# mhpi/hydrodl2

Hardware: AMD Instinct MI355X
Metric: basin-ensemble-timesteps/sec fwd+bwd (higher is better)
Workload: dtype f32

## Files before the change

hydrodl2_amd/csrc/hbv_chunked.h:

```cpp
#pragma once

#include <hip/hip_runtime.h>

#include "../../include/hbvx.h"
#include "hbv_step.h"

namespace hbvx {

struct ChunkArgs {
    hbvx_desc d;
    hbvx_bwd_io io;
    int lgMp;
    int C;
    int nchunk;
    float *phi;
    float *abnd;
    float *gpart;
    int nd;
    int dslot[3];
    int per_xcd;
};

struct ChunkBlock {
    int bx, chunk;
};
__host__ __device__ inline int chunk_per_xcd(int B, int lgMp)
{
    const int bpw = 64 >> lgMp;
    return ((B + bpw - 1) / bpw + 7) / 8;
}
__device__ __forceinline__ bool chunk_block(const hbvx_desc &d, int lgMp, int per_xcd, ChunkBlock &b)
{
    const int i = blockIdx.x;
#if defined(HBVX_CHUNK_XCD) && HBVX_CHUNK_XCD == 0
    b.chunk = i / (8 * per_xcd);
    b.bx = i - b.chunk * (8 * per_xcd);
#else
    const int c = i & 7, k = i >> 3;
    b.chunk = k / per_xcd;
    b.bx = c * per_xcd + (k - b.chunk * per_xcd);
#endif
    return b.bx * (64 >> lgMp) < d.B;
}

#define CHUNK_FEW 3

template <int NP>
__device__ __forceinline__ void slot_set(float *p, int slot, float v)
{
#pragma unroll
    for (int i = 0; i < NP; i++)
        if (slot == i) p[i] = v;
}
template <int NP>
__device__ __forceinline__ float slot_get(const float *p, int slot)
{
    float v = 0.0f;
#pragma unroll
    for (int i = 0; i < NP; i++)
        if (slot == i) v = p[i];
    return v;
}

struct ChunkLane {
    int jm, b, j;
    bool active, leader;
    int64_t n;
};

__device__ __forceinline__ ChunkLane chunk_lane(const hbvx_desc &d, int lgMp, int bx)
{
    ChunkLane L;
    const int lane = threadIdx.x & 63;
    const int Mp = 1 << lgMp;
    L.jm = lane & (Mp - 1);
    int b = bx * (64 >> lgMp) + (lane >> lgMp);
    L.active = (b < d.B) && (L.jm < d.M);
    L.leader = (b < d.B) && (L.jm == 0);
    L.b = b < d.B ? b : d.B - 1;
    L.j = L.jm < d.M ? L.jm : d.M - 1;
    L.n = (int64_t)L.b * d.M + L.j;
    return L;
}

template <int MODEL, bool BETAET>
struct ChunkNP {
    static constexpr int value = MODEL == MODEL_HBV10 ? (BETAET ? 13 : 12)
                               : MODEL == MODEL_HBV11P ? 14 : (MODEL == MODEL_HOURLY ? 19 : 16);
};

template <int NP>
struct ChunkRaw {
    float f[3];
    float st[5];
    float sw0, ef0;
    float gf[HBVX_MAX_FLUX];
    float g4[4];
    float dv[NP];
    float mu;
};

template <int MODEL, bool BETAET, int NP>
struct ChunkDay {
// ... 199 lines not shown
    const int chunk = blk.chunk;
    const int t0 = chunk * A.C, t1 = min(d.T, t0 + A.C);
    const int64_t N = (int64_t)d.B * d.M;
    const bool raw = d.raw_sigmoid != 0;
    const float nz = d.nearzero, invM = 1.0f / (float)d.M;
    const float ac = (MODEL == MODEL_HBV20 || MODEL == MODEL_HOURLY) ? d.ac[L.b] : 0.0f;
    const float elev = (MODEL == MODEL_HBV20 || MODEL == MODEL_HOURLY) ? d.elev[L.b] : 0.0f;
    float usta[NP], psta[NP];
    bool use_dyn[NP];
    chunk_static<NP, DYN>(d, L, raw, usta, psta, use_dyn, nd_, ds_);

    float Phi[5][5], phi[5];
#pragma unroll
    for (int k = 0; k < 5; k++) {
        phi[k] = 0.0f;
#pragma unroll
        for (int i = 0; i < 5; i++) Phi[k][i] = (i == k) ? 1.0f : 0.0f;
    }
    FluxGrad g0;
    g0.gQ = g0.gQ0 = g0.gQ1 = g0.gQ2 = g0.gET = g0.gSWE = g0.grech = g0.gexc = g0.gef = g0.gtosoil =
        g0.gPERC = g0.gcap = 0.0f;
    constexpr bool LDSDV = DYN == 3;
    __shared__ float dvbuf[LDSDV ? NP * 64 : 1];
    ChunkRaw<NP> Rn;
    if (LDSDV) chunk_dma_dyn<NP>(d, L, t1 - 1, dvbuf);
    chunk_issue<NP, DYN, GFULL, LDSDV, MU>(d, io, L, t1 - 1, io.n_flux, Rn, nd_, ds_);
    for (int t = t1 - 1; t >= t0; t--) {
        ChunkRaw<NP> Rc = Rn;
        if (LDSDV) {
            asm volatile("s_waitcnt vmcnt(0)" ::: "memory");
            chunk_pull_dyn<NP>(Rc, dvbuf);
            asm volatile("s_waitcnt lgkmcnt(0)" ::: "memory");
        }
        if (t > t0) {
            if (LDSDV) chunk_dma_dyn<NP>(d, L, t - 1, dvbuf);
            chunk_issue<NP, DYN, GFULL, LDSDV, MU>(d, io, L, t - 1, io.n_flux, Rn, nd_, ds_);
        }
        ChunkDay<MODEL, BETAET, NP> D;
        chunk_finish<MODEL, BETAET, NP, DYN, GFULL, MU>(d, Rc, raw, nz, ac, elev, usta, psta, use_dyn,
                                                    io.n_flux, invM, D, nd_, ds_, io.grad_flux4 != nullptr);
        float gp[NPARAM_MAX], gx[3];
#pragma unroll
        for (int i = 0; i < NPARAM_MAX; i++) gp[i] = 0.0f;
        if constexpr (MODEL == MODEL_HBV10) {
            typedef Step<MODEL, BETAET> S;
            const typename S::JT c = D.s.jt_coef(D.p, nz);
            S::template jt_unit<0>(c, Phi[0]);
            S::template jt_unit<0>(c, Phi[1]);
            S::template jt_unit<1>(c, Phi[2]);
            S::template jt_unit<2>(c, Phi[3]);
            S::template jt_unit<2>(c, Phi[4]);
            if constexpr (!GFULL) {
                S::jt_affine(c, phi, D.g.gQ0 + D.g.gQ, D.g.gQ1 + D.g.gQ, D.g.gQ2 + D.g.gQ);
                continue;
            }
        } else if constexpr (MODEL == MODEL_HBV11P || MODEL == MODEL_HBV20) {
            typedef Step<MODEL, BETAET> S;
            const typename S::JTC c = D.s.jt_coef_cap(D.p, nz);
            S::template jt_unit<0>(c, Phi[0]);
            S::template jt_unit<0>(c, Phi[1]);
#pragma unroll
            for (int k = 2; k < 5; k++) S::jt_cap(c, Phi[k], 0.0f, 0.0f, 0.0f);
            if constexpr (!GFULL) {
                S::jt_cap(c, phi, D.g.gQ0 + D.g.gQ, D.g.gQ1 + D.g.gQ, D.g.gQ2 + D.g.gQ);
                continue;
            }
        } else {
#pragma unroll
            for (int k = 0; k < 5; k++) D.s.bwd(D.p, nz, g0, Phi[k], gp, gx);
        }
        D.s.bwd(D.p, nz, D.g, phi, gp, gx);
    }
    if (L.active) {
        float *dst = A.phi + ((int64_t)chunk * 30) * N + L.n;
#pragma unroll
        for (int k = 0; k < 5; k++)
#pragma unroll
            for (int i = 0; i < 5; i++) dst[(int64_t)(k * 5 + i) * N] = Phi[k][i];
#pragma unroll
        for (int i = 0; i < 5; i++) dst[(int64_t)(25 + i) * N] = phi[i];
    }
}

__host__ __device__ constexpr int onepass_kmin(int i)
{
    return (i == P_TT || i == P_CFMAX || i == P_CFR || i == P_CWH) ? 0
         : ((i == P_BETA || i == P_FC || i == P_LP || i == P_BETAET) ? 2 : 3);
}
__host__ __device__ constexpr int onepass_row(int i)
{
    int r = 0;
    for (int j = 0; j < i; j++) r += 6 - onepass_kmin(j);
    return r;
}
__host__ __device__ constexpr int onepass_rows(int NP) { return onepass_row(NP); }

template <bool BETAET, bool GFULL>
__global__ void __launch_bounds__(64) k_bwd_chunk_onepass(const ChunkArgs A)
{
    constexpr int MODEL = MODEL_HBV10, DYN = 0;
    constexpr int NP = ChunkNP<MODEL, BETAET>::value;
    typedef Step<MODEL, BETAET> S;
    const int ds_[3] = {0, 0, 0};
    const hbvx_desc &d = A.d;
    const hbvx_bwd_io &io = A.io;
    ChunkBlock blk;
    if (!chunk_block(d, A.lgMp, A.per_xcd, blk)) return;
    const ChunkLane L = chunk_lane(d, A.lgMp, blk.bx);
    const int chunk = blk.chunk;
    const int t0 = chunk * A.C, t1 = min(d.T, t0 + A.C);
    const int64_t N = (int64_t)d.B * d.M;
    const bool raw = d.raw_sigmoid != 0;
    const float nz = d.nearzero, invM = 1.0f / (float)d.M;
    float usta[NP], psta[NP];
    bool use_dyn[NP];
    chunk_static<NP, DYN>(d, L, raw, usta, psta, use_dyn, 0, ds_);

    float Phi[5][5], phi[5];
    float G[6][NPARAM_MAX];
#pragma unroll
    for (int k = 0; k < 5; k++) {
        phi[k] = 0.0f;
#pragma unroll
        for (int i = 0; i < 5; i++) Phi[k][i] = (i == k) ? 1.0f : 0.0f;
    }
#pragma unroll
    for (int k = 0; k < 6; k++)
#pragma unroll
        for (int i = 0; i < NPARAM_MAX; i++) G[k][i] = 0.0f;
    ChunkRaw<NP> Rn;
    chunk_issue<NP, DYN, GFULL>(d, io, L, t1 - 1, io.n_flux, Rn, 0, ds_);
    for (int t = t1 - 1; t >= t0; t--) {
        ChunkRaw<NP> Rc = Rn;
        if (t > t0) chunk_issue<NP, DYN, GFULL>(d, io, L, t - 1, io.n_flux, Rn, 0, ds_);
        ChunkDay<MODEL, BETAET, NP> D;
        chunk_finish<MODEL, BETAET, NP, DYN, GFULL>(d, Rc, raw, nz, 0.0f, 0.0f, usta, psta, use_dyn, io.n_flux, invM,
                                                    D, 0, ds_, io.grad_flux4 != nullptr);
        const typename S::JT c = D.s.jt_coef(D.p, nz);
        const typename S::JG k = D.s.jg_coef(D.p, nz);
        S::template jt_gp<0>(c, k, Phi[0], G[0]);
        S::template jt_gp<0>(c, k, Phi[1], G[1]);
        S::template jt_gp<1>(c, k, Phi[2], G[2]);
        S::template jt_gp<2>(c, k, Phi[3], G[3]);
        S::template jt_gp<2>(c, k, Phi[4], G[4]);
        if constexpr (!GFULL) {
            S::template jt_gp<2, true>(c, k, phi, G[5], D.g.gQ0 + D.g.gQ, D.g.gQ1 + D.g.gQ, D.g.gQ2 + D.g.gQ);
        } else {
            float gx[3];
            D.s.bwd(D.p, nz, D.g, phi, G[5], gx);
        }
    }
    if (L.active) {
        float *dst = A.phi + ((int64_t)chunk * 30) * N + L.n;
#pragma unroll
        for (int k = 0; k < 5; k++)
#pragma unroll
            for (int i = 0; i < 5; i++) dst[(int64_t)(k * 5 + i) * N] = Phi[k][i];
#pragma unroll
        for (int i = 0; i < 5; i++) dst[(int64_t)(25 + i) * N] = phi[i];
        float *gdst = A.gpart + ((int64_t)chunk * onepass_rows(NP)) * N + L.n;
#pragma unroll
        for (int i = 0; i < NP; i++) {
            const int r0 = onepass_row(i), k0 = onepass_kmin(i);
#pragma unroll
            for (int kk = 0; kk < 5; kk++)
                if (kk >= k0) gdst[(int64_t)(r0 + kk - k0) * N] = G[kk][i];
            gdst[(int64_t)(r0 + 5 - k0) * N] = G[5][i];
        }
    }
}

#ifndef HBVX_CHUNK_NO_SHARED_KERNELS
__global__ void __launch_bounds__(64) k_bwd_chunk_scan(const ChunkArgs A)
{
    const hbvx_desc &d = A.d;
    const int64_t N = (int64_t)d.B * d.M;
    const int64_t n = (int64_t)blockIdx.x * 64 + threadIdx.x;
    if (n >= N) return;
    float a[5];
#pragma unroll
    for (int k = 0; k < 5; k++) a[k] = A.io.grad_state_out ? A.io.grad_state_out[k * N + n] : 0.0f;
    constexpr int SCAN_DEPTH = 4;
    float buf[SCAN_DEPTH][30];
    auto fetch = [&](int c, float *dst) __attribute__((always_inline)) {
        const float *src = A.phi + ((int64_t)c * 30) * N + n;
#pragma unroll
        for (int i = 0; i < 30; i++) dst[i] = src[(int64_t)i * N];
    };
#pragma unroll
    for (int j = 0; j < SCAN_DEPTH; j++)
        if (A.nchunk - 1 - j >= 0) fetch(A.nchunk - 1 - j, buf[j]);
    for (int c0 = A.nchunk - 1; c0 >= 0; c0 -= SCAN_DEPTH) {
#pragma unroll
        for (int j = 0; j < SCAN_DEPTH; j++) {
            const int c = c0 - j;
            if (c < 0) break;
            float cur[30];
#pragma unroll
            for (int i = 0; i < 30; i++) cur[i] = buf[j][i];
            if (c - SCAN_DEPTH >= 0) fetch(c - SCAN_DEPTH, buf[j]);
#pragma unroll
            for (int k = 0; k < 5; k++) A.abnd[((int64_t)c * 5 + k) * N + n] = a[k];
            float an[5];
#pragma unroll
            for (int i = 0; i < 5; i++) {
                float v = cur[25 + i];
#pragma unroll
                for (int k = 0; k < 5; k++) v += a[k] * cur[k * 5 + i];
                an[i] = v;
            }
#pragma unroll
            for (int i = 0; i < 5; i++) a[i] = an[i];
        }
    }
    if (A.io.grad_state_in) {
#pragma unroll
        for (int k = 0; k < 5; k++) A.io.grad_state_in[k * N + n] = a[k];
    }
}

#endif

__device__ __forceinline__ float chunk_ens_sum(float v, int lgMp)
{
    for (int s = 0; s < lgMp; s++) v += __shfl_xor(v, 1 << s, 64);
    return v;
}

template <int MODEL, bool BETAET, int DYN, bool GFULL, int SC = 0, bool ROWST = false, bool MU = false>
__global__ void __launch_bounds__(64) k_bwd_chunk_sweep(const ChunkArgs A)
{
    CHUNK_SLOTS(A);
    constexpr int NP = ChunkNP<MODEL, BETAET>::value;
    __shared__ float rowbuf[ROWST ? 64 * NP : 1];
    const hbvx_desc &d = A.d;
    const hbvx_bwd_io &io = A.io;
    ChunkBlock blk;
    if (!chunk_block(d, A.lgMp, A.per_xcd, blk)) return;
    const ChunkLane L = chunk_lane(d, A.lgMp, blk.bx);
    const int chunk = blk.chunk;
    const int t0 = chunk * A.C, t1 = min(d.T, t0 + A.C);
    const int64_t N = (int64_t)d.B * d.M;
    const bool raw = d.raw_sigmoid != 0;
    const float nz = d.nearzero, invM = 1.0f / (float)d.M;
    const float ac = (MODEL == MODEL_HBV20 || MODEL == MODEL_HOURLY) ? d.ac[L.b] : 0.0f;
    const float elev = (MODEL == MODEL_HBV20 || MODEL == MODEL_HOURLY) ? d.elev[L.b] : 0.0f;
    float usta[NP], psta[NP], gsta[NP];
    bool use_dyn[NP];
    chunk_static<NP, DYN>(d, L, raw, usta, psta, use_dyn, nd_, ds_);
#pragma unroll
    for (int i = 0; i < NP; i++) gsta[i] = 0.0f;
// ... 54 lines not shown
            const int M = d.M, rowf = NP * M, bl = (threadIdx.x & 63) >> A.lgMp;
            if (L.jm < M) {
#pragma unroll
                for (int i = 0; i < NP; i++) {
                    const float gu = gp[i] * (d.p[i].hi - d.p[i].lo);
                    rowbuf[bl * rowf + i * M + L.jm] = raw ? gu * (D.ud[i] * (1.0f - D.ud[i])) : gu;
                }
            }
            const int b0 = blk.bx * (64 >> A.lgMp);
            const int nb = min(64 >> A.lgMp, d.B - b0);
            const int half = rowf >> 1, total2 = nb * half;
            float *gbase = io.g[0].dyn + (int64_t)t * io.g[0].dyn_t_stride + (int64_t)b0 * io.g[0].dyn_b_stride;
            for (int k = threadIdx.x & 63; k < total2; k += 64) {
                const int rb = k / half, w2 = k - rb * half;
                const float2 v = *reinterpret_cast<const float2 *>(&rowbuf[rb * rowf + 2 * w2]);
                *reinterpret_cast<float2 *>(gbase + (int64_t)rb * io.g[0].dyn_b_stride + 2 * w2) = v;
            }
        }
#pragma unroll
        for (int i = 0; i < NP; i++) {
            if (DYN == 1 || DYN == 3) break;
            const float gu = gp[i] * (d.p[i].hi - d.p[i].lo);
            if (DYN == 2) {
                const float gr = raw ? gu * (D.ud[i] * (1.0f - D.ud[i])) : gu;
                if (io.g[i].dyn && L.active)
                    io.g[i].dyn[(int64_t)t * io.g[i].dyn_t_stride + (int64_t)L.b * io.g[i].dyn_b_stride + L.j] =
                        use_dyn[i] ? gr : 0.0f;
                gsta[i] += use_dyn[i] ? 0.0f : gu;
            } else {
                gsta[i] += gu;
            }
        }
        if (io.grad_x) {
            const float act = L.active ? 1.0f : 0.0f;
            const float g0 = chunk_ens_sum(gx[0] * act, A.lgMp), g1 = chunk_ens_sum(gx[1] * act, A.lgMp),
                        g2 = chunk_ens_sum(gx[2] * act, A.lgMp);
            if (L.leader) {
                float *gr = io.grad_x + (int64_t)t * d.x_t_stride + (int64_t)L.b * d.x_b_stride;
                gr[d.ch_prcp] = g0; gr[d.ch_tmean] = g1; gr[d.ch_pet] = g2;
            }
        }
    }
    if (DYN == 1) {
#pragma unroll
        for (int k = 0; k < CHUNK_FEW; k++)
            if (k < nd_) slot_set<NP>(gsta, ds_[k], slot_get<NP>(gsta, ds_[k]) - gused[k]);
    }
    if (DYN != 3 && L.active) {
#pragma unroll
        for (int i = 0; i < NP; i++) A.gpart[((int64_t)chunk * NP + i) * N + L.n] = gsta[i];
    }
}

#ifndef HBVX_CHUNK_NO_SHARED_KERNELS
__global__ void __launch_bounds__(256) k_bwd_chunk_reduce(const ChunkArgs A, int NP)
{
    const hbvx_desc &d = A.d;
    const hbvx_bwd_io &io = A.io;
    const int64_t N = (int64_t)d.B * d.M;
    const int64_t n = (int64_t)blockIdx.x * 256 + threadIdx.x;
    const int i = blockIdx.y;
    if (n >= N || !io.g[i].sta) return;
    const float *src = A.gpart + (int64_t)i * N + n;
    const int64_t cs = (int64_t)NP * N;
    float acc0 = 0.0f, acc1 = 0.0f, acc2 = 0.0f, acc3 = 0.0f;
    int c = 0;
    for (; c + 3 < A.nchunk; c += 4) {
        acc0 += src[(int64_t)c * cs];
        acc1 += src[(int64_t)(c + 1) * cs];
        acc2 += src[(int64_t)(c + 2) * cs];
        acc3 += src[(int64_t)(c + 3) * cs];
    }
    for (; c < A.nchunk; c++) acc0 += src[(int64_t)c * cs];
    float gsum = (acc0 + acc1) + (acc2 + acc3);
    const int b = (int)(n / d.M), j = (int)(n % d.M);
    if (d.raw_sigmoid) {
        const float u = sigmoid_(d.p[i].sta[(int64_t)b * d.p[i].sta_b_stride + j]);
        gsum = gsum * (u * (1.0f - u));
    }
    float *dst = io.g[i].sta + (int64_t)b * io.g[i].sta_b_stride + j;
    *dst += gsum;
}

#define ONEPASS_GROUP 4
template <int NP>
__global__ void __launch_bounds__(256) k_bwd_chunk_fold(const ChunkArgs A)
{
    constexpr int NR = onepass_rows(NP);
    const hbvx_desc &d = A.d;
    const int64_t N = (int64_t)d.B * d.M;
    const int64_t n = (int64_t)blockIdx.x * 256 + threadIdx.x;
    if (n >= N) return;
    const int grp = blockIdx.y;
    const int c0 = grp * ONEPASS_GROUP, c1 = min(A.nchunk, c0 + ONEPASS_GROUP);
    double acc[NP];
#pragma unroll
    for (int i = 0; i < NP; i++) acc[i] = 0.0;
    for (int c = c0; c < c1; c++) {
        const float *g = A.gpart + (int64_t)c * NR * N + n;
        const float *ab = A.abnd + (int64_t)c * 5 * N + n;
        double a[5];
#pragma unroll
        for (int k = 0; k < 5; k++) a[k] = ab[(int64_t)k * N];
#pragma unroll
        for (int i = 0; i < NP; i++) {
            const int k0 = onepass_kmin(i), r0 = onepass_row(i);
            double v = g[(int64_t)(r0 + 5 - k0) * N];
#pragma unroll
            for (int k = 0; k < 5; k++)
                if (k >= k0) v += (double)g[(int64_t)(r0 + k - k0) * N] * a[k];
            acc[i] += v;
        }
    }
    float *dst = A.phi + (int64_t)grp * NP * N + n;
#pragma unroll
    for (int i = 0; i < NP; i++) dst[(int64_t)i * N] = (float)acc[i] * (d.p[i].hi - d.p[i].lo);
}

#endif

}
```

hydrodl2_amd/csrc/launch_chunked.hip:

```cpp
#include "hbvx_host.h"
#include "hbv_chunked.h"

#include <algorithm>
#include <atomic>

using namespace hbvx;
using namespace hbvx_host;

namespace hbvx_host {
void launch_chunk_scan(const hbvx::ChunkArgs &a, hipStream_t st)
{
    const int64_t N = (int64_t)a.d.B * a.d.M;
    hipLaunchKernelGGL(k_bwd_chunk_scan, dim3((unsigned)((N + 63) / 64)), dim3(64), 0, st, a);
}
void launch_chunk_reduce(const hbvx::ChunkArgs &a, int n_param, hipStream_t st)
{
    const int64_t N = (int64_t)a.d.B * a.d.M;
    hipLaunchKernelGGL(k_bwd_chunk_reduce, dim3((unsigned)((N + 255) / 256), n_param), dim3(256), 0, st, a, n_param);
}
}

int hbvx_host::chunk_days() { int c = env_int("HBVX_CHUNK", 64); return c < 2 ? 2 : c; }

bool hbvx_host::chunked_applicable(const hbvx_desc *d)
{
    const char *v = getenv("HBVX_BWD");
    if (v && !strcmp(v, "tiled")) return false;
    return d->T >= 2 * chunk_days();
}

static int np_of(const hbvx_desc *d) { return d->n_param; }

static bool onepass_admitted(const hbvx_desc *d)
{
    return d->model == HBVX_MODEL_HBV10 && (d->n_param == 12 || d->n_param == 13) && count_dyn(d) == 0;
}

static int gpart_rows(const hbvx_desc *d)
{
    const int np = np_of(d);
    return onepass_admitted(d) ? std::max(np, onepass_rows(np)) : np;
}

extern "C" uint64_t hbvx_backward_workspace_bytes(const hbvx_desc *d)
{
    if (!d || d->T <= 0 || d->B <= 0 || d->M <= 0 || !chunked_applicable(d)) return 0;
    const int C = chunk_days();
    const uint64_t nchunk = (uint64_t)(d->T + C - 1) / C;
    return nchunk * (uint64_t)d->B * (uint64_t)d->M * (uint64_t)(35 + gpart_rows(d)) * sizeof(float);
}

static std::atomic<int> g_chunk_form{0};
extern "C" int hbvx_chunk_form(void) { return g_chunk_form.load(); }

template <int MODEL, bool BETAET, int DYN, bool GFULL>
static hipError_t launch_chunked_t(const ChunkArgs &a, hipStream_t st, bool onepass)
{
    const hbvx_desc &d = a.d;
    const int bpw = 64 >> a.lgMp;
    const int64_t N = (int64_t)d.B * d.M;
    (void)bpw;
    dim3 g2((unsigned)(8 * a.per_xcd * a.nchunk));
    if constexpr (MODEL == MODEL_HBV10 && DYN == 0) {
        if (onepass) {
            g_chunk_form = 1;
            hipLaunchKernelGGL((k_bwd_chunk_onepass<BETAET, GFULL>), g2, dim3(64), 0, st, a);
            hipLaunchKernelGGL(k_bwd_chunk_scan, dim3((unsigned)((N + 63) / 64)), dim3(64), 0, st, a);
            store_gate(&a.io, st);
            const int ngroup = (a.nchunk + ONEPASS_GROUP - 1) / ONEPASS_GROUP;
            hipLaunchKernelGGL((k_bwd_chunk_fold<ChunkNP<MODEL, BETAET>::value>),
                               dim3((unsigned)((N + 255) / 256), (unsigned)ngroup), dim3(256), 0, st, a);
            ChunkArgs r = a;
            r.gpart = a.phi;
            r.nchunk = ngroup;
            hipLaunchKernelGGL(k_bwd_chunk_reduce, dim3((unsigned)((N + 255) / 256), d.n_param), dim3(256), 0, st,
                               r, d.n_param);
            return hipGetLastError();
        }
    }
    g_chunk_form = 2;
    int sc = 0;
    const bool mu = d.muwts != nullptr;
    if (!mu && DYN == 1 && MODEL == MODEL_HBV10 && BETAET && a.nd == 2 && a.dslot[0] == P_BETA && a.dslot[1] == P_BETAET) sc = 1;
    if (!mu && DYN == 1 && (MODEL == MODEL_HBV20 || MODEL == MODEL_HOURLY) && a.nd == 3 && a.dslot[0] == P_BETA &&
        a.dslot[1] == P_K0 && a.dslot[2] == P_BETAET)
        sc = 2;
    if constexpr (DYN == 1 && MODEL == MODEL_HBV10 && BETAET) {
        if (sc == 1) {
            hipLaunchKernelGGL((k_bwd_chunk_phi<MODEL, BETAET, DYN, GFULL, 1>), g2, dim3(64), 0, st, a);
            hipLaunchKernelGGL(k_bwd_chunk_scan, dim3((unsigned)((N + 63) / 64)), dim3(64), 0, st, a);
            store_gate(&a.io, st);
            hipLaunchKernelGGL((k_bwd_chunk_sweep<MODEL, BETAET, DYN, GFULL, 1>), g2, dim3(64), 0, st, a);
        }
    }
    if constexpr (DYN == 1 && (MODEL == MODEL_HBV20 || MODEL == MODEL_HOURLY)) {
        if (sc == 2) {
            hipLaunchKernelGGL((k_bwd_chunk_phi<MODEL, BETAET, DYN, GFULL, 2>), g2, dim3(64), 0, st, a);
            hipLaunchKernelGGL(k_bwd_chunk_scan, dim3((unsigned)((N + 63) / 64)), dim3(64), 0, st, a);
            store_gate(&a.io, st);
            hipLaunchKernelGGL((k_bwd_chunk_sweep<MODEL, BETAET, DYN, GFULL, 2>), g2, dim3(64), 0, st, a);
        }
    }
    if (sc != 0) {
        hipLaunchKernelGGL(k_bwd_chunk_reduce, dim3((unsigned)((N + 255) / 256), d.n_param), dim3(256), 0, st,
                           a, d.n_param);
        return hipGetLastError();
    }
    if constexpr (DYN == 0 || DYN == 1) {
        if (d.muwts) {
            hipLaunchKernelGGL((k_bwd_chunk_phi<MODEL, BETAET, DYN, GFULL, 0, true>), g2, dim3(64), 0, st, a);
            hipLaunchKernelGGL(k_bwd_chunk_scan, dim3((unsigned)((N + 63) / 64)), dim3(64), 0, st, a);
            store_gate(&a.io, st);
            hipLaunchKernelGGL((k_bwd_chunk_sweep<MODEL, BETAET, DYN, GFULL, 0, false, true>), g2, dim3(64), 0, st, a);
            hipLaunchKernelGGL(k_bwd_chunk_reduce, dim3((unsigned)((N + 255) / 256), d.n_param), dim3(256), 0, st,
                               a, d.n_param);
            return hipGetLastError();
        }
    }
    hipLaunchKernelGGL((k_bwd_chunk_phi<MODEL, BETAET, DYN, GFULL>), g2, dim3(64), 0, st, a);
    hipLaunchKernelGGL(k_bwd_chunk_scan, dim3((unsigned)((N + 63) / 64)), dim3(64), 0, st, a);
    store_gate(&a.io, st);
    if constexpr (DYN == 3) {
        const hbvx_param_grad &g0 = a.io.g[0];
        bool rows = g0.dyn && ((uintptr_t)g0.dyn & 7) == 0 &&
                    (g0.dyn_b_stride & 1) == 0 && (g0.dyn_t_stride & 1) == 0 && ((d.n_param * d.M) & 1) == 0;
        for (int i = 1; i < d.n_param && rows; i++)
            rows = a.io.g[i].dyn == g0.dyn + (int64_t)i * d.M && a.io.g[i].dyn_b_stride == g0.dyn_b_stride &&
                   a.io.g[i].dyn_t_stride == g0.dyn_t_stride;
        if (rows) hipLaunchKernelGGL((k_bwd_chunk_sweep<MODEL, BETAET, DYN, GFULL, 0, true>), g2, dim3(64), 0, st, a);
        else hipLaunchKernelGGL((k_bwd_chunk_sweep<MODEL, BETAET, DYN, GFULL>), g2, dim3(64), 0, st, a);
        return hipGetLastError();
    }
    hipLaunchKernelGGL((k_bwd_chunk_sweep<MODEL, BETAET, DYN, GFULL>), g2, dim3(64), 0, st, a);
    if (DYN == 3) return hipGetLastError();
    hipLaunchKernelGGL(k_bwd_chunk_reduce, dim3((unsigned)((N + 255) / 256), d.n_param), dim3(256), 0, st,
                       a, d.n_param);
    return hipGetLastError();
}

template <int DYN, bool GFULL>
static hipError_t launch_chunked_v(const hbvx_desc *d, const ChunkArgs &a, hipStream_t st, bool onepass = false)
{
    return with_model(d, [&](auto m, auto be) { return launch_chunked_t<m, be, DYN, GFULL>(a, st, onepass); });
}

static hipError_t launch_chunked(const hbvx_desc *d, const hbvx_bwd_io *io, hipStream_t st)
{
    ChunkArgs a;
    a.d = *d;
    a.io = *io;
    a.lgMp = lg_members(d->M);
    a.C = chunk_days();
    a.nchunk = (d->T + a.C - 1) / a.C;
    a.per_xcd = chunk_per_xcd(d->B, a.lgMp);
    const int64_t N = (int64_t)d->B * d->M;
    a.phi = (float *)io->workspace;
    a.abnd = a.phi + (int64_t)a.nchunk * 30 * N;
    a.gpart = a.abnd + (int64_t)a.nchunk * 5 * N;
    const bool gfull = io->grad_flux != nullptr;
    a.nd = 0;
    a.dslot[0] = a.dslot[1] = a.dslot[2] = 0;
    const int ndyn = count_dyn(d);
    if (ndyn > 0 && ndyn <= CHUNK_FEW) {
        for (int i = 0; i < d->n_param; i++)
            if (d->p[i].dyn) a.dslot[a.nd++] = i;
        return gfull ? launch_chunked_v<1, true>(d, a, st) : launch_chunked_v<1, false>(d, a, st);
    }
    bool alldyn = ndyn == d->n_param && !d->muwts;
    for (int i = 0; i < d->n_param && alldyn; i++)
        alldyn = d->p[i].drop == nullptr && d->p[i].dyn == d->p[0].dyn + (int64_t)i * d->M &&
                 d->p[i].dyn_t_stride == d->p[0].dyn_t_stride && d->p[i].dyn_b_stride == d->p[0].dyn_b_stride;
    if (alldyn) return gfull ? launch_chunked_v<3, true>(d, a, st) : launch_chunked_v<3, false>(d, a, st);
    if (ndyn > 0) return gfull ? launch_chunked_v<2, true>(d, a, st) : launch_chunked_v<2, false>(d, a, st);
    const bool onepass = onepass_admitted(d) && !d->muwts && !io->grad_x && env_int("HBVX_CHUNK_ONEPASS", 1) != 0;
    return gfull ? launch_chunked_v<0, true>(d, a, st, onepass) : launch_chunked_v<0, false>(d, a, st, onepass);
}

bool hbvx_host::try_bwd_chunked(const hbvx_desc *d, const hbvx_bwd_io *io, void *stream, int *rc)
{
    if (io->workspace && chunked_applicable(d) && io->workspace_bytes >= hbvx_backward_workspace_bytes(d)) {
        hipError_t e = launch_chunked(d, io, (hipStream_t)stream);
        note_dispatch(1, "chunked");
        *rc = e != hipSuccess ? hip_fail(e, "hbvx_backward (chunked) launch") : HBVX_OK;
        return true;
    }
    return false;
}
```

hydrodl2_amd/csrc/launch_tiled.hip:

```cpp
#include "hbvx_host.h"
#include "hbv_tiled.h"
#define HBVX_CHUNK_NO_SHARED_KERNELS
#include "hbv_chunked.h"
#include "hbv_adj_kernels.h"

using namespace hbvx;
using namespace hbvx_host;

namespace hbvx_host {
void launch_chunk_scan(const hbvx::ChunkArgs &a, hipStream_t st);
void launch_chunk_reduce(const hbvx::ChunkArgs &a, int n_param, hipStream_t st);
}

static bool geom_fwd(const hbvx_desc *d, const hbvx_fwd_out *o, TileGeom &g)
{
    g = TileGeom{};
    g.lgMp = lg_members(d->M);
    g.ND = count_dyn(d);
    g.NDm = g.ND + (d->muwts ? 1 : 0);
    const int NF = (d->model == HBVX_MODEL_HBV10) ? 11 : (d->model == HBVX_MODEL_HBVADJ ? 1 : 12);
    const int wgs = (d->B + (64 >> g.lgMp) - 1) / (64 >> g.lgMp);
    const int ktmax = env_int("HBVX_KT", wgs >= 1024 ? 4 : 16);
    for (int Kt = 16; Kt >= 1; Kt >>= 1) {
        if (Kt > ktmax) continue;
// ... 93 lines not shown

static int check_adj(const hbvx_desc *d)
{
    int rc = check_desc(d);
    if (rc) return rc;
    if (d->model != HBVX_MODEL_HBVADJ) return fail(HBVX_E_UNSUPPORTED, "hbvx_adj_* needs model HBVADJ");
    if (!(d->adj_gtol >= 0.0f) || d->adj_max_iter < 0 || d->adj_max_iter > 64)
        return fail(HBVX_E_SHAPE, "bad Newton policy (adj_gtol / adj_max_iter)");
    return HBVX_OK;
}

static int adj_forward_dispatch(const hbvx_desc *d, const hbvx_fwd_out *out, void *stream);

extern "C" int hbvx_adj_forward(const hbvx_desc *d, const hbvx_fwd_out *out, void *stream)
{
    zero_taken() = false;
    if (out && out->zero_ptr && !out->zero_state) return fail(HBVX_E_NULL, "zero_ptr needs zero_state");
    return adj_forward_dispatch(d, out, stream);
}

static int adj_forward_dispatch(const hbvx_desc *d, const hbvx_fwd_out *out, void *stream)
{
    int rc = check_adj(d);
    if (rc) return rc;
    if (!out || !out->state_out) return fail(HBVX_E_NULL, "state_out is NULL");
    if (out->flux && out->n_flux != 1) return fail(HBVX_E_SHAPE, "hbvx_adj_forward writes n_flux = 1");
    if (d->adj_stop < 0 || d->adj_stop > 2) return fail(HBVX_E_SHAPE, "adj_stop must be 0, 1 or 2");
    if (d->adj_stop == 2 && try_fwd_pipe(d, out, stream, &rc)) return rc;
    {
        FwdTArgs ta;
        if (use_tiled(d) && geom_fwd(d, out, ta.g)) {
            ta.d = *d;
            ta.o = *out;
            const int bpw_t = 64 >> ta.g.lgMp;
            dim3 grid_t((d->B + bpw_t - 1) / bpw_t);
            const size_t lds = (size_t)2 * (ta.g.in_sz + ta.g.out_sz) * 4;
            const bool dyn = ta.g.NDm > 0, be = d->n_param == 13;
            int nh = env_int("HBVX_NH", 7);
            nh = nh < 1 ? 1 : (nh > 7 ? 7 : nh);
            const int threads = 64 * (1 + nh);
            hipStream_t st = (hipStream_t)stream;
            hipError_t e =
                be ? (dyn ? launch_tiled_one(k_fwd_tiled<MODEL_HBVADJ, true, true>, ta, grid_t, threads, lds, st)
                          : launch_tiled_one(k_fwd_tiled<MODEL_HBVADJ, true, false>, ta, grid_t, threads, lds, st))
                   : (dyn ? launch_tiled_one(k_fwd_tiled<MODEL_HBVADJ, false, true>, ta, grid_t, threads, lds, st)
                          : launch_tiled_one(k_fwd_tiled<MODEL_HBVADJ, false, false>, ta, grid_t, threads, lds, st));
            if (e != hipSuccess) return hip_fail(e, "hbvx_adj_forward (tiled) launch");
            return HBVX_OK;
        }
    }
    AdjFwdArgs a;
    a.d = *d;
    a.o = *out;
    a.lgMp = lg_members(d->M);
    const int bpw = 64 >> a.lgMp;
    dim3 grid((d->B + bpw - 1) / bpw);
    if (d->n_param == 13) hipLaunchKernelGGL(k_adj_fwd<true>, grid, dim3(64), 0, (hipStream_t)stream, a);
    else hipLaunchKernelGGL(k_adj_fwd<false>, grid, dim3(64), 0, (hipStream_t)stream, a);
    hipError_t e = hipGetLastError();
    if (e != hipSuccess) return hip_fail(e, "hbvx_adj_forward launch");
    return HBVX_OK;
}

extern "C" int hbvx_adj_backward(const hbvx_desc *d, const hbvx_bwd_io *io, void *stream)
{
    int rc = check_adj(d);
    if (rc) return rc;
    if (!io || !io->traj) return fail(HBVX_E_NULL, "traj is NULL");
    if (io->n_flux != 1) return fail(HBVX_E_SHAPE, "hbvx_adj_backward expects n_flux = 1");
    if (d->T == 0) return HBVX_OK;
    if (io->workspace && chunked_applicable(d) && io->workspace_bytes >= hbvx_backward_workspace_bytes(d)) {
        ChunkArgs ca;
        ca.d = *d;
        ca.io = *io;
        ca.lgMp = lg_members(d->M);
        ca.C = chunk_days();
        ca.nchunk = (d->T + ca.C - 1) / ca.C;
        const int64_t N = (int64_t)d->B * d->M;
        ca.phi = (float *)io->workspace;
        ca.abnd = ca.phi + (int64_t)ca.nchunk * 30 * N;
        ca.gpart = ca.abnd + (int64_t)ca.nchunk * 5 * N;
        hipStream_t st = (hipStream_t)stream;
        ca.per_xcd = chunk_per_xcd(d->B, ca.lgMp);
        dim3 g2((unsigned)(8 * ca.per_xcd * ca.nchunk));
        AdjFew few{};
        const bool is_few = count_dyn(d) <= ADJ_FEW;
        if (is_few)
            for (int i = 0; i < d->n_param; i++)
                if (d->p[i].dyn) few.slot[few.nd++] = i;
        if (d->n_param == 13) {
            if (is_few) hipLaunchKernelGGL((k_adj_chunk_phi<true, true>), g2, dim3(64), 0, st, *d, *io, ca.lgMp, ca.C, ca.phi, ca.per_xcd, few);
            else hipLaunchKernelGGL((k_adj_chunk_phi<true, false>), g2, dim3(64), 0, st, *d, *io, ca.lgMp, ca.C, ca.phi, ca.per_xcd, few);
        } else {
            if (is_few) hipLaunchKernelGGL((k_adj_chunk_phi<false, true>), g2, dim3(64), 0, st, *d, *io, ca.lgMp, ca.C, ca.phi, ca.per_xcd, few);
            else hipLaunchKernelGGL((k_adj_chunk_phi<false, false>), g2, dim3(64), 0, st, *d, *io, ca.lgMp, ca.C, ca.phi, ca.per_xcd, few);
        }
        launch_chunk_scan(ca, st);
        store_gate(io, st);
        if (d->n_param == 13) {
            if (is_few) hipLaunchKernelGGL((k_adj_chunk_sweep<true, true>), g2, dim3(64), 0, st, *d, *io, ca.lgMp, ca.C, ca.abnd, ca.gpart, ca.per_xcd, few);
            else hipLaunchKernelGGL((k_adj_chunk_sweep<true, false>), g2, dim3(64), 0, st, *d, *io, ca.lgMp, ca.C, ca.abnd, ca.gpart, ca.per_xcd, few);
        } else {
            if (is_few) hipLaunchKernelGGL((k_adj_chunk_sweep<false, true>), g2, dim3(64), 0, st, *d, *io, ca.lgMp, ca.C, ca.abnd, ca.gpart, ca.per_xcd, few);
            else hipLaunchKernelGGL((k_adj_chunk_sweep<false, false>), g2, dim3(64), 0, st, *d, *io, ca.lgMp, ca.C, ca.abnd, ca.gpart, ca.per_xcd, few);
        }
        launch_chunk_reduce(ca, d->n_param, st);
        hipError_t e = hipGetLastError();
        if (e != hipSuccess) return hip_fail(e, "hbvx_adj_backward (chunked) launch");
        return HBVX_OK;
    }
    AdjBwdArgs a;
    a.d = *d;
    a.io = *io;
    a.lgMp = lg_members(d->M);
    const int bpw = 64 >> a.lgMp;
    dim3 grid((d->B + bpw - 1) / bpw);
    store_gate(io, (hipStream_t)stream);
    if (d->n_param == 13) hipLaunchKernelGGL(k_adj_bwd<true>, grid, dim3(64), 0, (hipStream_t)stream, a);
    else hipLaunchKernelGGL(k_adj_bwd<false>, grid, dim3(64), 0, (hipStream_t)stream, a);
    hipError_t e = hipGetLastError();
    if (e != hipSuccess) return hip_fail(e, "hbvx_adj_backward launch");
    return HBVX_OK;
}

extern "C" int hbvx_adj_tangent_batch(const hbvx_desc *d, const hbvx_tan_batch *tb, const float *traj, void *stream)
{
    int rc = check_desc(d);
    if (rc) return rc;
    if (d->model != HBVX_MODEL_HBVADJ)
        return fail(HBVX_E_UNSUPPORTED, "hbvx_adj_tangent_batch: the implicit scheme (HBVADJ) only");
    if (!tb) return fail(HBVX_E_NULL, "tan_batch is NULL");
    if (tb->n_dir < 1) return fail(HBVX_E_SHAPE, "hbvx_adj_tangent_batch: n_dir must be >= 1");
    if (tb->n_dir > 65535) return fail(HBVX_E_SHAPE, "hbvx_adj_tangent_batch: too many directions for one launch");
    if (tb->n_flux != 1) return fail(HBVX_E_SHAPE, "hbvx_adj_tangent_batch: n_flux must be 1");
    if (tb->flux_mask >> tb->n_flux) return fail(HBVX_E_SHAPE, "flux_mask selects a series at or above n_flux");
    if (!traj) return fail(HBVX_E_NULL, "hbvx_adj_tangent_batch: traj is NULL (the trajectory of hbvx_adj_forward)");
    if (!tb->tan_state_out) return fail(HBVX_E_NULL, "tan_state_out is NULL");
    if (tb->flux_mask && !tb->tan_flux) return fail(HBVX_E_NULL, "tan_flux is NULL although flux_mask selects series");
    if (tb->muwts) return fail(HBVX_E_UNSUPPORTED, "hbvx_adj_tangent_batch: muwts must be NULL (the implicit scheme has no ensemble weights)");
    if (tb->dyn_t0 < 0 || tb->dyn_t0 > (d->T > 0 ? d->T - 1 : 0)) return fail(HBVX_E_SHAPE, "dyn_t0 outside the call's days");
    for (int i = d->n_param; i < HBVX_MAX_PARAM; i++)
        if (tb->p[i].dyn || tb->p[i].sta) return fail(HBVX_E_SHAPE, "tangent for a parameter slot the model lacks");
    for (int i = 0; i < d->n_param; i++)
        if (tb->p[i].dyn && !d->p[i].dyn) return fail(HBVX_E_SHAPE, "dynamic tangent for a static parameter");
    AdjTanArgs a;
    a.d = *d;
    a.tb = *tb;
    a.traj = traj;
    a.lgMp = lg_members(d->M);
    if (!a.tb.x_d_stride) a.tb.x = nullptr;
    if (!a.tb.state_d_stride) a.tb.state_in = nullptr;
    for (int i = 0; i < d->n_param; i++) {
        if (!a.tb.dyn_d_stride[i]) a.tb.p[i].dyn = nullptr;
        if (!a.tb.sta_d_stride[i]) a.tb.p[i].sta = nullptr;
    }
    const int bpw = 64 >> a.lgMp;
    const dim3 grid((d->B + bpw - 1) / bpw, (tb->n_dir + ADJ_TAN_G - 1) / ADJ_TAN_G);
    AdjFew few{};
    const bool is_few = count_dyn(d) <= ADJ_FEW;
    if (is_few)
        for (int i = 0; i < d->n_param; i++)
            if (d->p[i].dyn) few.slot[few.nd++] = i;
    hipStream_t st = (hipStream_t)stream;
    if (d->n_param == 13) {
        if (is_few) hipLaunchKernelGGL((k_adj_tan_batch<true, true>), grid, dim3(64), 0, st, a, few);
        else hipLaunchKernelGGL((k_adj_tan_batch<true, false>), grid, dim3(64), 0, st, a, few);
// ... 9 lines not shown
```

Before: 32.21 billion.

## Compose consecutive onepass chunk transfer matrices in-block via LDS before writing

The onepass backward kernel now runs up to four consecutive time chunks as separate waves of one block. Their per-chunk Jacobian products and parameter-gradient partials are composed through shared memory into a single group result, so only one slot per group goes to global memory. This cuts the global workspace writes and the work of the scan and fold kernels by the group factor, which defaults to four. The cost is extra block barriers and LDS traffic, serialized composition across waves, and changed waves-per-EU hints that may shift register allocation.

Result: faster. 34.49 billion (median of 6 runs) (+7.1%).

```diff
diff --git a/hydrodl2_amd/csrc/hbv_chunked.h b/hydrodl2_amd/csrc/hbv_chunked.h
--- a/hydrodl2_amd/csrc/hbv_chunked.h
+++ b/hydrodl2_amd/csrc/hbv_chunked.h
@@ -4,6 +4,7 @@
 
 #include "../../include/hbvx.h"
 #include "hbv_step.h"
+#include "hbv_onepass_compose.h"
 
 namespace hbvx {
 
@@ -19,6 +20,7 @@
     int nd;
     int dslot[3];
     int per_xcd;
+    int group;
 };
 
 struct ChunkBlock {
@@ -384,22 +386,37 @@
     }
 }
 
-__host__ __device__ constexpr int onepass_kmin(int i)
-{
-    return (i == P_TT || i == P_CFMAX || i == P_CFR || i == P_CWH) ? 0
-         : ((i == P_BETA || i == P_FC || i == P_LP || i == P_BETAET) ? 2 : 3);
-}
-__host__ __device__ constexpr int onepass_row(int i)
-{
-    int r = 0;
-    for (int j = 0; j < i; j++) r += 6 - onepass_kmin(j);
-    return r;
-}
-__host__ __device__ constexpr int onepass_rows(int NP) { return onepass_row(NP); }
+#define ONEPASS_GMAX 4
+__host__ __device__ constexpr int onepass_slot_bytes(int NP) { return (30 + onepass_rows(NP)) * 64 * (int)sizeof(float); }
+
+template <int NP>
+struct OnepassSlot {
+    float *s;
+    __device__ __forceinline__ float Phi(int k, int j) const { return s[(k * 5 + j) * 64]; }
+    __device__ __forceinline__ float phi(int j) const { return s[(25 + j) * 64]; }
+    __device__ __forceinline__ float G(int k, int p) const { return s[(30 + onepass_row(p) + k - onepass_kmin(p)) * 64]; }
+    __device__ __forceinline__ void Phi(int k, int i, float v) { s[(k * 5 + i) * 64] = v; }
+    __device__ __forceinline__ void phi(int i, float v) { s[(25 + i) * 64] = v; }
+    __device__ __forceinline__ void G(int k, int p, float v) { s[(30 + onepass_row(p) + k - onepass_kmin(p)) * 64] = v; }
+};
+template <int NP>
+struct OnepassRows {
+    float *m, *g;
+    int64_t N;
+    bool active;
+    __device__ __forceinline__ void Phi(int k, int i, float v) { if (active) m[(int64_t)(k * 5 + i) * N] = v; }
+    __device__ __forceinline__ void phi(int i, float v) { if (active) m[(int64_t)(25 + i) * N] = v; }
+    __device__ __forceinline__ void G(int k, int p, float v)
+    {
+        if (active) g[(int64_t)(onepass_row(p) + k - onepass_kmin(p)) * N] = v;
+    }
+};
 
 template <bool BETAET, bool GFULL>
-__global__ void __launch_bounds__(64) k_bwd_chunk_onepass(const ChunkArgs A)
-{
+__global__ void __launch_bounds__(64 * ONEPASS_GMAX) __attribute__((amdgpu_waves_per_eu(GFULL ? 2 : 3)))
+k_bwd_chunk_onepass(const ChunkArgs A)
+{
+    extern __shared__ float onepass_slot[];
     constexpr int MODEL = MODEL_HBV10, DYN = 0;
     constexpr int NP = ChunkNP<MODEL, BETAET>::value;
     typedef Step<MODEL, BETAET> S;
@@ -409,7 +426,10 @@
     ChunkBlock blk;
     if (!chunk_block(d, A.lgMp, A.per_xcd, blk)) return;
     const ChunkLane L = chunk_lane(d, A.lgMp, blk.bx);
-    const int chunk = blk.chunk;
+    const int grp = blk.chunk;
+    const int w = __builtin_amdgcn_readfirstlane((int)threadIdx.x >> 6);
+    const int nw = min(min(A.group, ONEPASS_GMAX), A.nchunk - grp * A.group);
+    const int chunk = grp * A.group + w;
     const int t0 = chunk * A.C, t1 = min(d.T, t0 + A.C);
     const int64_t N = (int64_t)d.B * d.M;
     const bool raw = d.raw_sigmoid != 0;
@@ -430,6 +450,7 @@
     for (int k = 0; k < 6; k++)
 #pragma unroll
         for (int i = 0; i < NPARAM_MAX; i++) G[k][i] = 0.0f;
+    if (w < nw) {
     ChunkRaw<NP> Rn;
     chunk_issue<NP, DYN, GFULL>(d, io, L, t1 - 1, io.n_flux, Rn, 0, ds_);
     for (int t = t1 - 1; t >= t0; t--) {
@@ -452,23 +473,28 @@
             D.s.bwd(D.p, nz, D.g, phi, G[5], gx);
         }
     }
-    if (L.active) {
-        float *dst = A.phi + ((int64_t)chunk * 30) * N + L.n;
-#pragma unroll
-        for (int k = 0; k < 5; k++)
-#pragma unroll
-            for (int i = 0; i < 5; i++) dst[(int64_t)(k * 5 + i) * N] = Phi[k][i];
-#pragma unroll
-        for (int i = 0; i < 5; i++) dst[(int64_t)(25 + i) * N] = phi[i];
-        float *gdst = A.gpart + ((int64_t)chunk * onepass_rows(NP)) * N + L.n;
-#pragma unroll
-        for (int i = 0; i < NP; i++) {
-            const int r0 = onepass_row(i), k0 = onepass_kmin(i);
-#pragma unroll
-            for (int kk = 0; kk < 5; kk++)
-                if (kk >= k0) gdst[(int64_t)(r0 + kk - k0) * N] = G[kk][i];
-            gdst[(int64_t)(r0 + 5 - k0) * N] = G[5][i];
-        }
+    }
+    OnepassRows<NP> rows{A.phi + ((int64_t)grp * 30) * N + L.n, A.gpart + ((int64_t)grp * onepass_rows(NP)) * N + L.n, N,
+                         L.active};
+    if (A.group == 1) {
+        onepass_put<float, NP>(Phi, phi, G, rows);
+        return;
+    }
+    OnepassSlot<NP> slot{onepass_slot + (threadIdx.x & 63)};
+    if (w == nw - 1 && w > 0) onepass_put<float, NP>(Phi, phi, G, slot);
+    static_assert(ONEPASS_GMAX == 4, "one stage per wave above wave 0");
+    if (nw > 1) {
+        if (nw > 2) {
+            if (nw > 3) __syncthreads();
+            if (w == 2 && nw > 3) onepass_compose<float, NP, false>(slot, Phi, phi, G, slot);
+            __syncthreads();
+        }
+        if (w == 1 && nw > 2) onepass_compose<float, NP, false>(slot, Phi, phi, G, slot);
+        __syncthreads();
+    }
+    if (w == 0) {
+        if (nw == 1) onepass_put<float, NP>(Phi, phi, G, rows);
+        else onepass_compose<float, NP, true>(slot, Phi, phi, G, rows);
     }
 }
 
@@ -689,7 +715,7 @@
     *dst += gsum;
 }
 
-#define ONEPASS_GROUP 4
+#define ONEPASS_FOLD_GROUP 4
 template <int NP>
 __global__ void __launch_bounds__(256) k_bwd_chunk_fold(const ChunkArgs A)
 {
@@ -699,7 +725,7 @@
     const int64_t n = (int64_t)blockIdx.x * 256 + threadIdx.x;
     if (n >= N) return;
     const int grp = blockIdx.y;
-    const int c0 = grp * ONEPASS_GROUP, c1 = min(A.nchunk, c0 + ONEPASS_GROUP);
+    const int c0 = grp * ONEPASS_FOLD_GROUP, c1 = min(A.nchunk, c0 + ONEPASS_FOLD_GROUP);
     double acc[NP];
 #pragma unroll
     for (int i = 0; i < NP; i++) acc[i] = 0.0;
diff --git a/hydrodl2_amd/csrc/hbv_onepass_compose.h b/hydrodl2_amd/csrc/hbv_onepass_compose.h
--- /dev/null
+++ b/hydrodl2_amd/csrc/hbv_onepass_compose.h
@@ -0,0 +1,117 @@
+#pragma once
+
+#include "hbv_step.h"
+
+#if defined(__HIPCC__)
+#define HBVX_HDC __host__ __device__ constexpr
+#else
+#define HBVX_HDC constexpr
+#endif
+#if defined(__HIP_DEVICE_COMPILE__)
+#define HBVX_SCHED_FENCE() __builtin_amdgcn_sched_barrier(0)
+#else
+#define HBVX_SCHED_FENCE() ((void)0)
+#endif
+
+namespace hbvx {
+
+HBVX_HDC int onepass_kmin(int i)
+{
+    return (i == P_TT || i == P_CFMAX || i == P_CFR || i == P_CWH) ? 0
+         : ((i == P_BETA || i == P_FC || i == P_LP || i == P_BETAET) ? 2 : 3);
+}
+HBVX_HDC int onepass_row(int i)
+{
+    int r = 0;
+    for (int j = 0; j < i; j++) r += 6 - onepass_kmin(j);
+    return r;
+}
+HBVX_HDC int onepass_rows(int NP) { return onepass_row(NP); }
+HBVX_HDC int onepass_reach(int k) { return k < 2 ? 2 : (k == 2 ? 3 : 5); }
+
+template <typename T, int NP, typename Dst>
+HBVX_HDM void onepass_put(const T Phi[5][5], const T phi[5], const T G[6][NPARAM_MAX], Dst &out)
+{
+#pragma unroll
+    for (int k = 0; k < 5; k++) {
+        out.phi(k, phi[k]);
+#pragma unroll
+        for (int i = 0; i < 5; i++) out.Phi(k, i, Phi[k][i]);
+    }
+#pragma unroll
+    for (int p = 0; p < NP; p++)
+#pragma unroll
+        for (int k = onepass_kmin(p); k < 6; k++) out.G(k, p, G[k][p]);
+}
+
+template <typename T, int NP, bool DENSE, typename Src, typename Dst>
+HBVX_HDM void onepass_compose(const Src &L, const T Phi[5][5], const T phi[5], const T G[6][NPARAM_MAX], Dst &out)
+{
+    T PL[5][5], pl[5];
+#pragma unroll
+    for (int k = 0; k < 5; k++) {
+        pl[k] = L.phi(k);
+#pragma unroll
+        for (int j = 0; j < 5; j++) PL[k][j] = j < onepass_reach(k) ? L.Phi(k, j) : T(0);
+    }
+    HBVX_SCHED_FENCE();
+#pragma unroll
+    for (int i = 0; i < 5; i++) {
+        T v = phi[i];
+#pragma unroll
+        for (int j = 0; j < 5; j++)
+            if (i < onepass_reach(j)) v += pl[j] * Phi[j][i];
+        out.phi(i, v);
+#pragma unroll
+        for (int k = 0; k < 5; k++) {
+            if (i >= onepass_reach(k)) {
+                if (DENSE) out.Phi(k, i, T(0));
+                continue;
+            }
+            T s = T(0);
+            bool first = true;
+#pragma unroll
+            for (int j = 0; j < 5; j++)
+                if (j < onepass_reach(k) && i < onepass_reach(j)) {
+                    s = first ? PL[k][j] * Phi[j][i] : s + PL[k][j] * Phi[j][i];
+                    first = false;
+                }
+            out.Phi(k, i, s);
+        }
+    }
+    T ln[6];
+#pragma unroll
+    for (int k = 0; k < 6; k++) ln[k] = k >= onepass_kmin(0) ? L.G(k, 0) : T(0);
+    HBVX_SCHED_FENCE();
+#pragma unroll
+    for (int p = 0; p < NP; p++) {
+        const int k0 = onepass_kmin(p);
+        T lc[6];
+#pragma unroll
+        for (int k = 0; k < 6; k++) lc[k] = ln[k];
+        if (p + 1 < NP) {
+#pragma unroll
+            for (int k = 0; k < 6; k++) ln[k] = k >= onepass_kmin(p + 1) ? L.G(k, p + 1) : T(0);
+        }
+        double ge[5];
+#pragma unroll
+        for (int j = 0; j < 5; j++) ge[j] = j >= k0 ? (double)G[j][p] : 0.0;
+        double v0 = (double)lc[5] + (double)G[5][p];
+#pragma unroll
+        for (int j = 0; j < 5; j++)
+            if (j >= k0) v0 = fma((double)pl[j], ge[j], v0);
+        out.G(5, p, (T)v0);
+#pragma unroll
+        for (int k = 0; k < 5; k++) {
+            if (k < k0) continue;
+            double v = (double)lc[k];
+#pragma unroll
+            for (int j = 0; j < 5; j++)
+                if (j >= k0 && j < onepass_reach(k)) v = fma((double)PL[k][j], ge[j], v);
+            out.G(k, p, (T)v);
+        }
+        HBVX_SCHED_FENCE();
+    }
+}
+
+}
diff --git a/hydrodl2_amd/csrc/launch_chunked.hip b/hydrodl2_amd/csrc/launch_chunked.hip
--- a/hydrodl2_amd/csrc/launch_chunked.hip
+++ b/hydrodl2_amd/csrc/launch_chunked.hip
@@ -52,6 +52,12 @@
 
 static std::atomic<int> g_chunk_form{0};
 extern "C" int hbvx_chunk_form(void) { return g_chunk_form.load(); }
+
+#define ONEPASS_GROUP_DEFAULT 4
+static int onepass_group() { return std::min(std::max(env_int("HBVX_ONEPASS_GROUP", ONEPASS_GROUP_DEFAULT), 1), ONEPASS_GMAX); }
+static std::atomic<int> g_onepass_group{0};
+extern "C" int hbvx_onepass_group(void) { return g_onepass_group.load(); }
+extern "C" int hbvx_onepass_slot_bytes(int n_param) { return onepass_slot_bytes(n_param); }
 
 template <int MODEL, bool BETAET, int DYN, bool GFULL>
 static hipError_t launch_chunked_t(const ChunkArgs &a, hipStream_t st, bool onepass)
@@ -63,13 +69,21 @@
     dim3 g2((unsigned)(8 * a.per_xcd * a.nchunk));
     if constexpr (MODEL == MODEL_HBV10 && DYN == 0) {
         if (onepass) {
+            constexpr int NP = ChunkNP<MODEL, BETAET>::value;
             g_chunk_form = 1;
-            hipLaunchKernelGGL((k_bwd_chunk_onepass<BETAET, GFULL>), g2, dim3(64), 0, st, a);
-            hipLaunchKernelGGL(k_bwd_chunk_scan, dim3((unsigned)((N + 63) / 64)), dim3(64), 0, st, a);
-            store_gate(&a.io, st);
-            const int ngroup = (a.nchunk + ONEPASS_GROUP - 1) / ONEPASS_GROUP;
-            hipLaunchKernelGGL((k_bwd_chunk_fold<ChunkNP<MODEL, BETAET>::value>),
-                               dim3((unsigned)((N + 255) / 256), (unsigned)ngroup), dim3(256), 0, st, a);
+            ChunkArgs o = a;
+            o.group = onepass_group();
+            g_onepass_group = o.group;
+            const int ngrp = (a.nchunk + o.group - 1) / o.group;
+            hipLaunchKernelGGL((k_bwd_chunk_onepass<BETAET, GFULL>), dim3((unsigned)(8 * a.per_xcd * ngrp)),
+                               dim3(64 * o.group), o.group > 1 ? onepass_slot_bytes(NP) : 0, st, o);
+            ChunkArgs s = a;
+            s.nchunk = ngrp;
+            hipLaunchKernelGGL(k_bwd_chunk_scan, dim3((unsigned)((N + 63) / 64)), dim3(64), 0, st, s);
+            store_gate(&a.io, st);
+            const int ngroup = (ngrp + ONEPASS_FOLD_GROUP - 1) / ONEPASS_FOLD_GROUP;
+            hipLaunchKernelGGL((k_bwd_chunk_fold<NP>), dim3((unsigned)((N + 255) / 256), (unsigned)ngroup), dim3(256), 0,
+                               st, s);
             ChunkArgs r = a;
             r.gpart = a.phi;
             r.nchunk = ngroup;
@@ -153,6 +167,7 @@
     a.C = chunk_days();
     a.nchunk = (d->T + a.C - 1) / a.C;
     a.per_xcd = chunk_per_xcd(d->B, a.lgMp);
+    a.group = 1;
     const int64_t N = (int64_t)d->B * d->M;
     a.phi = (float *)io->workspace;
     a.abnd = a.phi + (int64_t)a.nchunk * 30 * N;
diff --git a/hydrodl2_amd/csrc/launch_tiled.hip b/hydrodl2_amd/csrc/launch_tiled.hip
--- a/hydrodl2_amd/csrc/launch_tiled.hip
+++ b/hydrodl2_amd/csrc/launch_tiled.hip
@@ -199,6 +199,7 @@
         ca.gpart = ca.abnd + (int64_t)ca.nchunk * 5 * N;
         hipStream_t st = (hipStream_t)stream;
         ca.per_xcd = chunk_per_xcd(d->B, ca.lgMp);
+        ca.group = 1;
         dim3 g2((unsigned)(8 * ca.per_xcd * ca.nchunk));
         AdjFew few{};
         const bool is_few = count_dyn(d) <= ADJ_FEW;
```
